# bioinformatics-ua/polus

Measured on AMD Instinct MI355X. Metric: train samples/sec BioBERT-base NER seq256, higher is better.
Workload: dtype bf16; 1 GPU; BERT-base (L=12,H=768,A=12,I=3072,V=28996) token classification C=4, seq_len=256, 64 samples/GPU, AdamW lr 5e-5 wd 0.01 warm-up 10%, dropout 0.1 (hidden + attention) (BASELINE.json configs[2] per-GPU shape), random-init weights; global_batch=64, seq_len=256, parallelism=dp1, grad_allreduce=none

## Files before the change

polus_amd/csrc/common.h:

```cpp
#pragma once
#include <hip/hip_runtime.h>
#include <stdint.h>
#include <stdio.h>
#include <string.h>
#include <math.h>

#include "../../include/polus_hip.h"

typedef __bf16 bf16_t;
typedef __bf16 bf16x8 __attribute__((ext_vector_type(8)));
typedef __bf16 bf16x4 __attribute__((ext_vector_type(4)));
typedef short s16x4 __attribute__((ext_vector_type(4)));
typedef float f32x4 __attribute__((ext_vector_type(4)));

void polus_set_error(const char* fmt, ...);
#define POLUS_FAIL(...) do { polus_set_error(__VA_ARGS__); return POLUS_ERR_INVALID; } while (0)
#define POLUS_REQUIRE(cond, ...) do { if (!(cond)) { polus_set_error(__VA_ARGS__); return POLUS_ERR_INVALID; } } while (0)
#define POLUS_CHECK_LAUNCH(name) do { hipError_t e__ = hipGetLastError(); \
    if (e__ != hipSuccess) { polus_set_error("%s: launch failed: %s", name, hipGetErrorString(e__)); return POLUS_ERR_HIP; } } while (0)
#define POLUS_HIP(call) do { hipError_t e__ = (call); \
    if (e__ != hipSuccess) { polus_set_error("%s failed: %s", #call, hipGetErrorString(e__)); return POLUS_ERR_HIP; } } while (0)

template <auto Kern, typename... A>
int polus_launch_lds(const char* who, dim3 grid, dim3 block, size_t lds_max, size_t lds, hipStream_t st, const A&... args) {
    static bool attr_done = false;
    if (!attr_done) {
        POLUS_HIP(hipFuncSetAttribute(reinterpret_cast<const void*>(Kern), hipFuncAttributeMaxDynamicSharedMemorySize, (int)lds_max));
        attr_done = true;
    }
    hipLaunchKernelGGL(Kern, grid, block, lds, st, args...);
    POLUS_CHECK_LAUNCH(who);
    return POLUS_OK;
}

static inline size_t polus_dtype_size(int dt) { return dt == POLUS_BF16 ? 2 : 4; }
static inline bool polus_aligned16(const void* p) { return (((uintptr_t)p) & 15) == 0; }

struct PolusCfg {
    int gemm_pp;
    int gemm_v1;
    int dw_ungrouped;
    int dw_fused_reduce;
    int ln_bwd_blocks;
    int ln_fin_single;
    int gemm_ring128;
    int gemm_auto_split;
    int ln_halfwave;
    int gemm_order;
    int gemm_persist;
    int reserve_cus;
    int attn_bwd_kres;
    int attn_debug;
    int attn_kskip;
    int dw_streamk;
    int dw_sk_cus;
    int dw_sk_delta;
    int attn_fused;
};
const PolusCfg& polus_cfg();
int polus_num_cus();
int polus_reserved_cus();

struct PolusDyn { uint32_t salt; float lr, lr_t; uint32_t pad; };
const PolusDyn* polus_dyn();
__device__ __forceinline__ uint32_t polus_eff_seed(uint32_t seed, const PolusDyn* dyn) {
    if (!dyn) return seed;
    uint32_t x = seed + dyn->salt;
    x ^= x >> 15;
    return x * 0x2C1B3C6Du;
}

template <typename T> __device__ __forceinline__ float to_f(T x);
template <> __device__ __forceinline__ float to_f<float>(float x) { return x; }
template <> __device__ __forceinline__ float to_f<bf16_t>(bf16_t x) { return (float)x; }
template <typename T> __device__ __forceinline__ T from_f(float x);
template <> __device__ __forceinline__ float from_f<float>(float x) { return x; }
template <> __device__ __forceinline__ bf16_t from_f<bf16_t>(float x) { return (bf16_t)x; }

template <typename T> __device__ __forceinline__ void load4(const T* p, float (&v)[4]);
template <> __device__ __forceinline__ void load4<float>(const float* p, float (&v)[4]) {
    float4 t = *reinterpret_cast<const float4*>(p); v[0] = t.x; v[1] = t.y; v[2] = t.z; v[3] = t.w;
}
template <> __device__ __forceinline__ void load4<bf16_t>(const bf16_t* p, float (&v)[4]) {
    bf16x4 t = *reinterpret_cast<const bf16x4*>(p);
    v[0] = (float)t[0]; v[1] = (float)t[1]; v[2] = (float)t[2]; v[3] = (float)t[3];
}
template <typename T> __device__ __forceinline__ void store4(T* p, const float (&v)[4]);
template <> __device__ __forceinline__ void store4<float>(float* p, const float (&v)[4]) {
    *reinterpret_cast<float4*>(p) = make_float4(v[0], v[1], v[2], v[3]);
}
template <> __device__ __forceinline__ void store4<bf16_t>(bf16_t* p, const float (&v)[4]) {
    bf16x4 t; t[0] = (bf16_t)v[0]; t[1] = (bf16_t)v[1]; t[2] = (bf16_t)v[2]; t[3] = (bf16_t)v[3];
    *reinterpret_cast<bf16x4*>(p) = t;
}

__device__ __forceinline__ float erf_fast(float x) {
    const float ax = fabsf(x);
    const float t = __frcp_rn(1.0f + 0.3275911f * ax);
    float poly = 1.061405429f;
    poly = poly * t - 1.453152027f;
    poly = poly * t + 1.421413741f;
    poly = poly * t - 0.284496736f;
    poly = poly * t + 0.254829592f;
    const float r = 1.0f - poly * t * __expf(-ax * ax);
    return copysignf(r, x);
}
__device__ __forceinline__ float gelu_f(float x) { return 0.5f * x * (1.0f + erf_fast(x * 0.70710678118654752f)); }
__device__ __forceinline__ float gelu_grad_f(float x) {
    float cdf = 0.5f * (1.0f + erf_fast(x * 0.70710678118654752f));
    float pdf = 0.3989422804014327f * __expf(-0.5f * x * x);
    return cdf + x * pdf;
}
__device__ __forceinline__ float swish_f(float x) { return x / (1.0f + __expf(-x)); }
__device__ __forceinline__ float swish_grad_f(float x) {
    float s = 1.0f / (1.0f + __expf(-x));
    return s * (1.0f + x * (1.0f - s));
}
typedef float f32x2_t __attribute__((ext_vector_type(2)));
__device__ __forceinline__ f32x2_t gelu_poly2(f32x2_t x, const float (&c)[11]) {
    f32x2_t xc = {__builtin_amdgcn_fmed3f(x[0], -4.5f, 4.5f), __builtin_amdgcn_fmed3f(x[1], -4.5f, 4.5f)};
    f32x2_t s = xc * xc;
    f32x2_t u = __builtin_elementwise_fma(s, (f32x2_t){2.0f / 20.25f, 2.0f / 20.25f}, (f32x2_t){-1.0f, -1.0f});
    f32x2_t r = {c[10], c[10]};
#pragma unroll
    for (int k = 9; k >= 0; --k) r = __builtin_elementwise_fma(r, u, (f32x2_t){c[k], c[k]});
    return __builtin_elementwise_fma(xc, r, (f32x2_t){0.5f, 0.5f});
}
__device__ __forceinline__ f32x2_t gelu_cdf2(f32x2_t x) {
    const float q[11] = {1.569049305e-01f, -7.719386095e-02f, 5.470119065e-02f, -4.010921159e-02f, 2.828393083e-02f,
                         -1.902094059e-02f, 1.143922652e-02f, -5.251548121e-03f, 2.716277400e-03f, -2.340015935e-03f,
                         9.806926012e-04f};
    return gelu_poly2(x, q);
}
__device__ __forceinline__ f32x2_t gelu_grad2(f32x2_t x) {
    const float w[11] = {1.594289755e-01f, -9.003904569e-02f, 8.714168751e-02f, -9.350841452e-02f, 9.645831298e-02f,
                         -9.557466143e-02f, 7.437658385e-02f, -3.356380937e-02f, 2.252388123e-02f, -3.068672777e-02f,
                         1.457471506e-02f};
    return gelu_poly2(x, w);
}
template <int N, bool FAST = false> __device__ __forceinline__ void apply_act_n(int act, float (&v)[N]) {
    if (act == POLUS_ACT_GELU) {
        if (FAST && (N % 2) == 0) {
#pragma unroll
            for (int r = 0; r < N; r += 2) {
                f32x2_t x = {v[r], v[r + 1]};
                f32x2_t y = x * gelu_cdf2(x);
                v[r] = y[0]; v[r + 1] = y[1];
            }
            return;
        }
#pragma unroll
        for (int r = 0; r < N; ++r) v[r] = gelu_f(v[r]);
    } else if (act == POLUS_ACT_SWISH) {
#pragma unroll
        for (int r = 0; r < N; ++r) v[r] = swish_f(v[r]);
    } else if (act == POLUS_ACT_RELU) {
#pragma unroll
        for (int r = 0; r < N; ++r) v[r] = fmaxf(v[r], 0.0f);
    } else if (act == POLUS_ACT_TANH) {
#pragma unroll
        for (int r = 0; r < N; ++r) v[r] = tanhf(v[r]);
    }
}
template <int N, bool FAST = false> __device__ __forceinline__ void apply_act_grad_n(int act, float (&v)[N], const float (&u)[N]) {
    if (act == POLUS_ACT_GELU) {
        if (FAST && (N % 2) == 0) {
#pragma unroll
            for (int r = 0; r < N; r += 2) {
                f32x2_t d = (f32x2_t){v[r], v[r + 1]} * gelu_grad2((f32x2_t){u[r], u[r + 1]});
                v[r] = d[0]; v[r + 1] = d[1];
            }
            return;
        }
#pragma unroll
        for (int r = 0; r < N; ++r) v[r] *= gelu_grad_f(u[r]);
    } else if (act == POLUS_ACT_SWISH) {
#pragma unroll
        for (int r = 0; r < N; ++r) v[r] *= swish_grad_f(u[r]);
    } else if (act == POLUS_ACT_RELU) {
#pragma unroll
        for (int r = 0; r < N; ++r) v[r] = u[r] > 0.0f ? v[r] : 0.0f;
    } else if (act == POLUS_ACT_TANH) {
#pragma unroll
        for (int r = 0; r < N; ++r) { float t = tanhf(u[r]); v[r] *= 1.0f - t * t; }
    }
}

__device__ __forceinline__ uint32_t polus_hash32(uint32_t seed, uint32_t idx) {
    uint32_t x = idx * 0x9E3779B1u + seed;
    x ^= x >> 16; x *= 0x85EBCA6Bu;
    x ^= x >> 13; x *= 0xC2B2AE35u;
    x ^= x >> 16;
    return x;
}
__device__ __forceinline__ uint32_t polus_hash32_second(uint32_t h1) {
    uint32_t y = h1 * 0x27D4EB2Fu;
    return y ^ (y >> 15);
}
__device__ __forceinline__ bool polus_keep(uint32_t seed, uint32_t idx, uint32_t thresh) {
    const uint32_t h1 = polus_hash32(seed, idx >> 2);
    const uint32_t h = (idx & 2u) ? polus_hash32_second(h1) : h1;
    return ((idx & 1u) ? (h >> 16) : (h & 0xFFFFu)) >= thresh;
}
__device__ __forceinline__ void polus_keep4(uint32_t seed, uint32_t idx4, uint32_t thresh, bool (&k)[4]) {
    const uint32_t h1 = polus_hash32(seed, idx4 >> 2), h2 = polus_hash32_second(h1);
    k[0] = (h1 & 0xFFFFu) >= thresh;
    k[1] = (h1 >> 16) >= thresh;
    k[2] = (h2 & 0xFFFFu) >= thresh;
    k[3] = (h2 >> 16) >= thresh;
}
template <int N>
__device__ __forceinline__ void polus_dropout_run(float (&v)[N], uint32_t seed, uint32_t base, uint32_t thresh, float inv, bool quad) {
    static_assert(N % 4 == 0, "runs of whole quads");
    if (quad) {
#pragma unroll
        for (int r = 0; r < N; r += 4) {
            bool k[4];
            polus_keep4(seed, base + r, thresh, k);
#pragma unroll
            for (int e = 0; e < 4; ++e) v[r + e] = k[e] ? v[r + e] * inv : 0.f;
        }
    } else {
#pragma unroll
        for (int r = 0; r < N; ++r) v[r] = polus_keep(seed, base + r, thresh) ? v[r] * inv : 0.f;
    }
}
static inline uint32_t polus_drop_thresh(float p) {
    double t = (double)p * 65536.0 + 0.5;
    return t <= 0.0 ? 0u : (t >= 65535.0 ? 65535u : (uint32_t)t);
}

__device__ __forceinline__ float wave_sum(float v) {
#pragma unroll
    for (int o = 32; o > 0; o >>= 1) v += __shfl_xor(v, o, 64);
    return v;
}
__device__ __forceinline__ float wave_max(float v) {
#pragma unroll
    for (int o = 32; o > 0; o >>= 1) v = fmaxf(v, __shfl_xor(v, o, 64));
    return v;
}

template <typename T> struct Frag;
template <> struct Frag<bf16_t> { bf16x8 v; };
template <> struct Frag<float> { float v[8]; };

__device__ __forceinline__ void mma16(f32x4& acc, const Frag<bf16_t>& a, const Frag<bf16_t>& b) {
    acc = __builtin_amdgcn_mfma_f32_16x16x32_bf16(a.v, b.v, acc, 0, 0, 0);
}
__device__ __forceinline__ void mma16(f32x4& acc, const Frag<float>& a, const Frag<float>& b) {
#pragma unroll
    for (int j = 0; j < 8; ++j) acc = __builtin_amdgcn_mfma_f32_16x16x4f32(a.v[j], b.v[j], acc, 0, 0, 0);
}

typedef __attribute__((address_space(3))) s16x4 lds_s16x4;

__device__ __forceinline__ void frag_load_row(Frag<bf16_t>& f, const unsigned char* p) {
    f.v = *reinterpret_cast<const bf16x8*>(p);
}
__device__ __forceinline__ void frag_load_row(Frag<float>& f, const unsigned char* p) {
    float4 a = *reinterpret_cast<const float4*>(p);
    float4 b = *reinterpret_cast<const float4*>(p + 16);
    f.v[0] = a.x; f.v[1] = a.y; f.v[2] = a.z; f.v[3] = a.w;
    f.v[4] = b.x; f.v[5] = b.y; f.v[6] = b.z; f.v[7] = b.w;
}

__device__ __forceinline__ s16x4 lds_tr16(const unsigned char* p) {
    return __builtin_amdgcn_ds_read_tr16_b64_v4i16((lds_s16x4*)(p));
}
```

polus_amd/csrc/embed.hip:

```cpp
#include "rowwise.h"

namespace {

template <int NC>
__device__ __forceinline__ void gather_sum(const float* word, const float* pos, const float* type, int id, int s,
                                           int tt, int H, int lane, float (&v)[NC][4]) {
    const float* w = word + (long)id * H;
    const float* p = pos + (long)s * H;
    const float* t = type + (long)tt * H;
#pragma unroll
    for (int c = 0; c < NC; ++c) {
        int col = (lane + 64 * c) * 4;
        if (col < H) {
            float a[4], b[4], d[4];
            load4<float>(w + col, a); load4<float>(p + col, b); load4<float>(t + col, d);
#pragma unroll
            for (int e = 0; e < 4; ++e) v[c][e] = (a[e] + d[e]) + b[e];
        } else { v[c][0] = v[c][1] = v[c][2] = v[c][3] = 0.f; }
    }
}

template <typename T, int NC>
__global__ __launch_bounds__(LN_THREADS) void embed_fwd_kernel(const int32_t* __restrict__ ids, const int32_t* __restrict__ tts,
                                                        const float* __restrict__ word, const float* __restrict__ pos,
                                                        const float* __restrict__ type, const float* __restrict__ gamma,
                                                        const float* __restrict__ beta, T* __restrict__ y,
                                                        float* __restrict__ mean, float* __restrict__ rstd,
                                                        int B, int S, int H, int vocab, int type_vocab, float eps,
                                                        unsigned dthresh, unsigned dseed, float dinv, const PolusDyn* dyn) {
    if (dthresh) dseed = polus_eff_seed(dseed, dyn);
    const int lane = threadIdx.x & 63, wid = threadIdx.x >> 6;
    const int rows = B * S;
    float gv[NC][4], bv[NC][4];
    load_feat<NC>(gamma, H, lane, gv);
    load_feat<NC>(beta, H, lane, bv);
    for (int row = blockIdx.x * WAVES + wid; row < rows; row += gridDim.x * WAVES) {
        const int id = clamp_id(ids[row], vocab);
        const int tt = clamp_id(tts ? tts[row] : 0, type_vocab);
        float v[NC][4];
        gather_sum<NC>(word, pos, type, id, row % S, tt, H, lane, v);
        float mu, rs;
        row_stats<NC>(v, H, lane, eps, mu, rs);
        normalize_store<T, NC>(v, gv, bv, y + (long)row * H, H, lane, mu, rs, dthresh, dseed, dinv, (unsigned)row * (unsigned)H);
        if (lane == 0) { mean[row] = mu; rstd[row] = rs; }
    }
}

template <typename T, int NC>
__global__ __launch_bounds__(LN_THREADS) void embed_bwd_ln_kernel(const T* __restrict__ dy, const int32_t* __restrict__ ids,
                                                           const int32_t* __restrict__ tts, const float* __restrict__ word,
                                                           const float* __restrict__ pos, const float* __restrict__ type,
                                                           const float* __restrict__ gamma, const float* __restrict__ mean,
                                                           const float* __restrict__ rstd, float* __restrict__ de,
                                                           float* __restrict__ partial, int B, int S, int H, int vocab,
                                                           int type_vocab, DropArgs in_drop) {
    if (in_drop.thresh) in_drop.seed = polus_eff_seed(in_drop.seed, in_drop.dyn);
    extern __shared__ __attribute__((aligned(16))) unsigned char smem_raw[];
    float* lds = reinterpret_cast<float*>(smem_raw);
    const int lane = threadIdx.x & 63, wid = threadIdx.x >> 6;
    const int rows = B * S;
    ColAcc<NC> acc;
    colacc_zero(acc);
    float gv[NC][4];
    load_feat<NC>(gamma, H, lane, gv);
    for (int row = blockIdx.x * WAVES + wid; row < rows; row += gridDim.x * WAVES) {
        const int id = clamp_id(ids[row], vocab);
        const int tt = clamp_id(tts ? tts[row] : 0, type_vocab);
        float xv[NC][4];
        gather_sum<NC>(word, pos, type, id, row % S, tt, H, lane, xv);
        ln_bwd_row<T, float, NC>(xv, dy + (long)row * H, gv, de + (long)row * H, H, lane, mean[row], rstd[row], acc, 0,
                                 nullptr, DropArgs{0, 0, 1.f}, in_drop, (unsigned)row * (unsigned)H);
    }
    colacc_flush(acc, lds, partial, H, lane, wid, 0);
}

constexpr int SC_RUN = 8, SC_WAVES = 8;
template <int NC>
__global__ __launch_bounds__(64 * SC_WAVES) void embed_scatter_atomic_kernel(const float* __restrict__ de, const int32_t* __restrict__ ids,
                                                                      float* __restrict__ gword, int rows, int H, int vocab) {
    const int lane = threadIdx.x & 63, wid = threadIdx.x >> 6;
    const long stride = (long)gridDim.x * SC_WAVES * SC_RUN;
    for (long r0 = ((long)blockIdx.x * SC_WAVES + wid) * SC_RUN; r0 < rows; r0 += stride) {
        int mine = -1;
        if (lane < SC_RUN && r0 + lane < rows) mine = clamp_id(ids[r0 + lane], vocab);
        float row[SC_RUN][NC][4];
#pragma unroll
        for (int j = 0; j < SC_RUN; ++j) {
            const bool valid = r0 + j < rows;
            const float* src = de + (r0 + j) * H + lane;
#pragma unroll
            for (int c = 0; c < NC; ++c)
#pragma unroll
                for (int k = 0; k < 4; ++k)
                    row[j][c][k] = (valid && c * 256 + k * 64 + lane < H) ? src[c * 256 + k * 64] : 0.f;
        }
#pragma unroll
        for (int t = 0; t < SC_RUN; ++t) {
            const int id = __shfl(mine, t, 64);
            const unsigned same = (unsigned)__ballot(mine == id);
            if (id < 0 || (same & ((1u << t) - 1u))) continue;
            float* dst = gword + (long)id * H + lane;
#pragma unroll
            for (int c = 0; c < NC; ++c)
#pragma unroll
                for (int k = 0; k < 4; ++k) {
                    float acc = row[t][c][k];
#pragma unroll
                    for (int j = t + 1; j < SC_RUN; ++j)
                        if ((same >> j) & 1u) acc += row[j][c][k];
                    if (c * 256 + k * 64 + lane < H) atomicAdd(dst + c * 256 + k * 64, acc);
                }
        }
    }
}
__global__ __launch_bounds__(LN_THREADS) void embed_scatter_atomic_wide_kernel(const float* __restrict__ de, const int32_t* __restrict__ ids,
                                                                        float* __restrict__ gword, int rows, int H, int vocab) {
    const int lane = threadIdx.x & 63, wid = threadIdx.x >> 6;
    for (int row = blockIdx.x * WAVES + wid; row < rows; row += gridDim.x * WAVES) {
        const int id = clamp_id(ids[row], vocab);
        const float* src = de + (long)row * H;
        float* dst = gword + (long)id * H;
        for (int col = lane; col < H; col += 64) atomicAdd(dst + col, src[col]);
    }
}

__global__ __launch_bounds__(LN_THREADS) void embed_scatter_owner_kernel(const float* __restrict__ de, const int32_t* __restrict__ ids,
                                                                  float* __restrict__ gword, int rows, int H, int vocab) {
    const int lane = threadIdx.x & 63, wid = threadIdx.x >> 6;
    for (int row = blockIdx.x * WAVES + wid; row < rows; row += gridDim.x * WAVES) {
        auto clampid = [vocab](int v) { return clamp_id(v, vocab); };
        const int cid = clampid(ids[row]);
        bool dup = false;
        for (int j0 = 0; j0 < row && !dup; j0 += 64) {
            int j = j0 + lane;
            bool hit = (j < row) && (clampid(ids[j]) == cid);
            dup = __any(hit);
        }
        if (dup) continue;
        float* dst = gword + (long)cid * H;
        for (int c0 = 0; c0 < H; c0 += 64 * 4) {
            int col = c0 + lane * 4;
            float a[4] = {0.f, 0.f, 0.f, 0.f};
            for (int j0 = row; j0 < rows; j0 += 64) {
                int j = j0 + lane;
                unsigned long long m = __ballot((j < rows) && (clampid(ids[j]) == cid));
                while (m) {
                    int b = __ffsll((long long)m) - 1;
                    m &= m - 1;
                    if (col < H) {
                        float v[4];
                        load4<float>(de + (long)(j0 + b) * H + col, v);
#pragma unroll
                        for (int e = 0; e < 4; ++e) a[e] += v[e];
                    }
                }
            }
            if (col < H) {
                float o[4];
                load4<float>(dst + col, o);
#pragma unroll
                for (int e = 0; e < 4; ++e) o[e] += a[e];
                store4<float>(dst + col, o);
            }
        }
    }
}

__global__ __launch_bounds__(256) void embed_pos_grad_kernel(const float* __restrict__ de, float* __restrict__ gpos,
                                                             int B, int S, int H, int accumulate) {
    long idx = (long)blockIdx.x * blockDim.x + threadIdx.x;
    if (idx >= (long)S * H) return;
    float s = 0.f;
    for (int b = 0; b < B; ++b) s += de[(long)b * S * H + idx];
    gpos[idx] = accumulate ? gpos[idx] + s : s;
}

}

extern "C" size_t polus_embed_bwd_workspace_bytes(int B, int S, int H) {
    size_t rows = (size_t)B * S;
    size_t de = rows * H * sizeof(float);
    size_t part = polus_layernorm_bwd_workspace_bytes((int)rows, H);
    size_t cs = polus_colsum_workspace_bytes((int)rows, H);
    return de + (part > cs ? part : cs) + 256;
}

extern "C" int polus_embed_ln_fwd(int dtype, const int32_t* ids, const int32_t* type_ids,
                                  const float* word, const float* pos, const float* type,
                                  const float* gamma, const float* beta, void* y, float* mean, float* rstd,
                                  int B, int S, int H, int vocab, int max_pos, int type_vocab, float eps,
                                  float drop_p, uint32_t seed, void* stream) {
    POLUS_REQUIRE(ids && word && pos && type && gamma && beta && y && mean && rstd, "polus_embed_ln_fwd: null pointer");
    POLUS_REQUIRE(rowwise_drop_ok(drop_p, (long)B * S, H), "polus_embed_ln_fwd: bad drop_p");
    POLUS_REQUIRE(B > 0 && S > 0 && S <= max_pos, "polus_embed_ln_fwd: S=%d exceeds max_position_embeddings=%d", S, max_pos);
    POLUS_REQUIRE(rowwise_shape_ok((long)B * S, H) && vocab > 0 && type_vocab > 0, "polus_embed_ln_fwd: bad H=%d", H);
    POLUS_REQUIRE(polus_aligned16(word) && polus_aligned16(pos) && polus_aligned16(type) && polus_aligned16(y) &&
                  polus_aligned16(gamma) && polus_aligned16(beta), "polus_embed_ln_fwd: pointers must be 16-byte aligned");
    hipStream_t st = static_cast<hipStream_t>(stream);
    const DropArgs d = drop_args(drop_p, seed);
    const dim3 grid(row_blocks(B * S));
    POLUS_REQUIRE(dtype == POLUS_BF16 || dtype == POLUS_F32, "polus_embed_ln_fwd: bad dtype");
    for_dtype_chunks<1, 2, 3, 4, 8>(dtype, chunks256(H), [&](auto t, auto nc) {
        using T = decltype(t);
        hipLaunchKernelGGL((embed_fwd_kernel<T, nc()>), grid, dim3(LN_THREADS), 0, st, ids, type_ids, word, pos, type, gamma, beta, (T*)y, mean, rstd, B, S, H, vocab, type_vocab, eps, d.thresh, d.seed, d.inv, d.dyn);
    });
    POLUS_CHECK_LAUNCH("polus_embed_ln_fwd");
    return POLUS_OK;
}

extern "C" int polus_embed_ln_bwd(int dtype, const void* dy, const int32_t* ids, const int32_t* type_ids,
                                  const float* word, const float* pos, const float* type, const float* gamma,
                                  const float* mean, const float* rstd,
                                  float* gword, float* gpos, float* gtype, float* ggamma, float* gbeta,
                                  int accumulate, int deterministic,
                                  int B, int S, int H, int vocab, int max_pos, int type_vocab,
                                  float drop_p, uint32_t seed,
                                  void* workspace, size_t workspace_bytes, void* stream) {
    POLUS_REQUIRE(dy && ids && word && pos && type && gamma && mean && rstd && gword && gpos && gtype && ggamma && gbeta,
                  "polus_embed_ln_bwd: null pointer");
    POLUS_REQUIRE(rowwise_drop_ok(drop_p, (long)B * S, H), "polus_embed_ln_bwd: bad drop_p");
    POLUS_REQUIRE(B > 0 && S > 0 && S <= max_pos && rowwise_shape_ok((long)B * S, H), "polus_embed_ln_bwd: bad shape");
    POLUS_REQUIRE(polus_aligned16(dy) && polus_aligned16(gword) && polus_aligned16(workspace),
                  "polus_embed_ln_bwd: pointers must be 16-byte aligned");
    size_t need = polus_embed_bwd_workspace_bytes(B, S, H);
    if (!workspace || workspace_bytes < need) { polus_set_error("polus_embed_ln_bwd: workspace %zu < %zu", workspace_bytes, need); return POLUS_ERR_WORKSPACE; }
    hipStream_t st = static_cast<hipStream_t>(stream);
    const DropArgs in_drop = drop_args(drop_p, seed);
    const int rows = B * S;
    float* de = static_cast<float*>(workspace);
    size_t de_bytes = ((size_t)rows * H * sizeof(float) + 255) / 256 * 256;
    float* partial = reinterpret_cast<float*>(static_cast<unsigned char*>(workspace) + de_bytes);
    size_t partial_bytes = workspace_bytes - de_bytes;
    const int blocks = ln_blocks(rows);
    const size_t lds = 3 * (size_t)H * sizeof(float);
    POLUS_REQUIRE(dtype == POLUS_BF16 || dtype == POLUS_F32, "polus_embed_ln_bwd: bad dtype");
    for_dtype_chunks<1, 2, 3, 4, 8>(dtype, chunks256(H), [&](auto t, auto nc) {
        using T = decltype(t);
        hipLaunchKernelGGL((embed_bwd_ln_kernel<T, nc()>), dim3(blocks), dim3(LN_THREADS), lds, st, (const T*)dy, ids, type_ids, word, pos, type, gamma, mean, rstd, de, partial, B, S, H, vocab, type_vocab, in_drop);
    });
    POLUS_CHECK_LAUNCH("polus_embed_ln_bwd(ln)");
    int rc = polus_ln_finalize(partial, blocks, H, 0, ggamma, gbeta, nullptr, accumulate, 1, st, "polus_embed_ln_bwd(finalize)");
    if (rc != POLUS_OK) return rc;

    if (!accumulate) {
        POLUS_HIP(hipMemsetAsync(gword, 0, (size_t)vocab * H * sizeof(float), st));
        POLUS_HIP(hipMemsetAsync(gpos, 0, (size_t)max_pos * H * sizeof(float), st));
    }
    const int route = scatter_route(H, deterministic);
    if (route == SCATTER_OWNER)
        hipLaunchKernelGGL(embed_scatter_owner_kernel, dim3(row_blocks(rows)), dim3(LN_THREADS), 0, st, de, ids, gword, rows, H, vocab);
    else if (route == SCATTER_WIDE)
        hipLaunchKernelGGL(embed_scatter_atomic_wide_kernel, dim3(row_blocks(rows)), dim3(LN_THREADS), 0, st, de, ids, gword, rows, H, vocab);
    else
        for_chunks<1, 2, 3, 4>(route, [&](auto nc) {
            hipLaunchKernelGGL(embed_scatter_atomic_kernel<nc()>, dim3(capped_blocks(rows, SC_RUN * SC_WAVES, ROW_GRID_CAP)), dim3(64 * SC_WAVES), 0, st, de, ids, gword, rows, H, vocab);
        });
    POLUS_CHECK_LAUNCH("polus_embed_ln_bwd(scatter)");
    hipLaunchKernelGGL(embed_pos_grad_kernel, dim3(((long)S * H + 255) / 256), dim3(256), 0, st, de, gpos, B, S, H, accumulate);
    POLUS_CHECK_LAUNCH("polus_embed_ln_bwd(pos)");
    for (int t = 0; t < type_vocab; ++t) {
        if (type_ids || t == 0) {
            rc = polus_colsum_launch(POLUS_F32, de, H, rows, H, gtype + (long)t * H, accumulate, type_ids, t, partial, partial_bytes, st);
            if (rc != POLUS_OK) return rc;
        } else if (!accumulate) {
            POLUS_HIP(hipMemsetAsync(gtype + (long)t * H, 0, (size_t)H * sizeof(float), st));
        }
    }
    return POLUS_OK;
}
```

polus_amd/csrc/runtime.hip:

```cpp
#include "common.h"
#include <stdarg.h>

static thread_local char g_err[512] = "";

void polus_set_error(const char* fmt, ...) {
    va_list ap;
    va_start(ap, fmt);
    vsnprintf(g_err, sizeof(g_err), fmt, ap);
    va_end(ap);
}

extern "C" const char* polus_last_error(void) { return g_err; }

static PolusCfg g_cfg;
static bool g_cfg_ready = false;
static int env_int(const char* name, int dflt) {
    const char* e = getenv(name);
    return (e && *e) ? atoi(e) : dflt;
}
static void read_cfg() {
    g_cfg.gemm_pp = env_int("POLUS_GEMM_PP", 0);
    g_cfg.gemm_v1 = getenv("POLUS_GEMM_V1") != nullptr;
    g_cfg.dw_ungrouped = getenv("POLUS_DW_UNGROUPED") != nullptr;
    g_cfg.gemm_order = env_int("POLUS_GEMM_ORDER", 4);
    g_cfg.reserve_cus = env_int("POLUS_GEMM_RESERVE_CUS", 0);
    g_cfg.gemm_persist = env_int("POLUS_GEMM_PERSIST", 1);
    g_cfg.dw_fused_reduce = env_int("POLUS_DW_FUSED_REDUCE", 1);
    g_cfg.attn_fused = env_int("POLUS_ATTN_FUSED", 1);
    g_cfg.attn_bwd_kres = env_int("POLUS_ATTN_BWD_KRES", 1);
    g_cfg.attn_debug = env_int("POLUS_ATTN_DEBUG", 0);
    g_cfg.attn_kskip = env_int("POLUS_ATTN_KSKIP", 1);
    g_cfg.ln_halfwave = env_int("POLUS_LN_HALFWAVE", 1);
    g_cfg.gemm_auto_split = env_int("POLUS_GEMM_AUTO_SPLIT", 1);
    g_cfg.gemm_ring128 = env_int("POLUS_GEMM_RING128", 0);
    g_cfg.ln_bwd_blocks = env_int("POLUS_LN_BWD_BLOCKS", 512);
    g_cfg.ln_fin_single = env_int("POLUS_LN_FIN_SINGLE", 512);
    g_cfg.dw_streamk = env_int("POLUS_DW_STREAMK", 0);
    g_cfg.dw_sk_delta = env_int("POLUS_DW_SK_DELTA", 2);
    g_cfg.dw_sk_cus = env_int("POLUS_DW_SK_CUS", 0);
    g_cfg_ready = true;
}
const PolusCfg& polus_cfg() {
    if (!g_cfg_ready) read_cfg();
    return g_cfg;
}
extern "C" int polus_reload_env(void) { read_cfg(); return POLUS_OK; }

int polus_num_cus() {
    static int n = 0;
    if (!n) {
        int dev = 0; hipDeviceProp_t prop;
        if (hipGetDevice(&dev) == hipSuccess && hipGetDeviceProperties(&prop, dev) == hipSuccess) n = prop.multiProcessorCount;
        if (n <= 0) n = 256;
    }
    return n;
}
static int g_reserve_on = 1;
extern "C" int polus_set_reserve_active(int on) { g_reserve_on = on != 0; return POLUS_OK; }
int polus_reserved_cus() { return g_reserve_on ? polus_cfg().reserve_cus : 0; }

static const PolusDyn* g_dyn = nullptr;
const PolusDyn* polus_dyn() { return g_dyn; }
extern "C" int polus_set_dynamic_params(const void* dev_block16) {
    POLUS_REQUIRE(dev_block16 == nullptr || polus_aligned16(dev_block16), "polus_set_dynamic_params: the block must be 16-byte aligned");
    g_dyn = static_cast<const PolusDyn*>(dev_block16);
    return POLUS_OK;
}
extern "C" int polus_abi_version(void) { return POLUS_ABI_VERSION; }

extern "C" int polus_device_info(int* n_cu, int* lds_bytes_per_cu, char* arch, int arch_len) {
    int dev = 0;
    POLUS_HIP(hipGetDevice(&dev));
    hipDeviceProp_t prop;
    POLUS_HIP(hipGetDeviceProperties(&prop, dev));
    if (n_cu) *n_cu = prop.multiProcessorCount;
    if (lds_bytes_per_cu) *lds_bytes_per_cu = (int)prop.maxSharedMemoryPerMultiProcessor;
    if (arch && arch_len > 0) {
        strncpy(arch, prop.gcnArchName, arch_len - 1);
        arch[arch_len - 1] = 0;
    }
    return POLUS_OK;
}

namespace {

template <typename S, typename D>
__global__ void cast_kernel(const S* __restrict__ src, D* __restrict__ dst, int64_t n) {
    int64_t i4 = ((int64_t)blockIdx.x * blockDim.x + threadIdx.x) * 4;
    const int64_t stride = (int64_t)gridDim.x * blockDim.x * 4;
    for (; i4 < n; i4 += stride) {
        if (i4 + 4 <= n) {
            float v[4];
            load4<S>(src + i4, v);
            store4<D>(dst + i4, v);
        } else {
            for (int64_t j = i4; j < n; ++j) dst[j] = from_f<D>(to_f<S>(src[j]));
        }
    }
}

__global__ void scale_kernel(float* __restrict__ x, float a, int64_t n) {
    int64_t i4 = ((int64_t)blockIdx.x * blockDim.x + threadIdx.x) * 4;
    const int64_t stride = (int64_t)gridDim.x * blockDim.x * 4;
    for (; i4 < n; i4 += stride) {
        if (i4 + 4 <= n) {
            float4 v = *reinterpret_cast<float4*>(x + i4);
            v.x *= a; v.y *= a; v.z *= a; v.w *= a;
            *reinterpret_cast<float4*>(x + i4) = v;
        } else {
            for (int64_t j = i4; j < n; ++j) x[j] *= a;
        }
    }
}

template <typename T>
__global__ void act_bwd_kernel(const T* __restrict__ dy, const T* __restrict__ u, T* __restrict__ du, int64_t n, int act) {
    int64_t i4 = ((int64_t)blockIdx.x * blockDim.x + threadIdx.x) * 4;
    const int64_t stride = (int64_t)gridDim.x * blockDim.x * 4;
    for (; i4 < n; i4 += stride) {
        if (i4 + 4 <= n) {
            float a[4], b[4];
            load4<T>(dy + i4, a);
            load4<T>(u + i4, b);
            apply_act_grad_n<4>(act, a, b);
            store4<T>(du + i4, a);
        } else {
            for (int64_t j = i4; j < n; ++j) { float a1[1] = {to_f<T>(dy[j])}, b1[1] = {to_f<T>(u[j])}; apply_act_grad_n<1>(act, a1, b1); du[j] = from_f<T>(a1[0]); }
        }
    }
}

__global__ __launch_bounds__(256) void transpose16_kernel(const unsigned short* __restrict__ src,
                                                         unsigned short* __restrict__ dst, int R, int C) {
    __shared__ unsigned short tile[64][66];
    const int r0 = blockIdx.y * 64, c0 = blockIdx.x * 64;
    const int tx = threadIdx.x & 63, ty = threadIdx.x >> 6;
    for (int k = ty; k < 64; k += 4) {
        int r = r0 + k, c = c0 + tx;
        tile[k][tx] = (r < R && c < C) ? src[(long)r * C + c] : (unsigned short)0;
    }
    __syncthreads();
    for (int k = ty; k < 64; k += 4) {
        int c = c0 + k, r = r0 + tx;
        if (c < C && r < R) dst[(long)c * R + r] = tile[tx][k];
    }
}

__global__ __launch_bounds__(256) void transpose16_batched_kernel(const unsigned short* __restrict__ src,
                                                                 unsigned short* __restrict__ dst,
                                                                 const long* __restrict__ segs, int nseg) {
    __shared__ unsigned short tile[64][66];
    const int b = blockIdx.x;
    int s = 0;
    while (s + 1 < nseg && segs[4 * (s + 1) + 3] <= b) ++s;
    const long off = segs[4 * s];
    const int R = (int)segs[4 * s + 1], C = (int)segs[4 * s + 2];
    const int t = b - (int)segs[4 * s + 3], tc = (C + 63) / 64;
    const int r0 = (t / tc) * 64, c0 = (t % tc) * 64;
    const unsigned short* sp = src + off;
    unsigned short* dp = dst + off;
    if (((R | C) & 3) == 0) {
        const int q = threadIdx.x & 15, rr = threadIdx.x >> 4;
#pragma unroll
        for (int k = 0; k < 4; ++k) {
            const int r = r0 + rr + 16 * k, c = c0 + 4 * q;
            ushort4 v = make_ushort4(0, 0, 0, 0);
            if (r < R && c < C) v = *reinterpret_cast<const ushort4*>(sp + (long)r * C + c);
            tile[rr + 16 * k][4 * q] = v.x; tile[rr + 16 * k][4 * q + 1] = v.y;
            tile[rr + 16 * k][4 * q + 2] = v.z; tile[rr + 16 * k][4 * q + 3] = v.w;
        }
        __syncthreads();
#pragma unroll
        for (int k = 0; k < 4; ++k) {
            const int c = c0 + rr + 16 * k, r = r0 + 4 * q;
            if (c < C && r < R) {
                ushort4 v = make_ushort4(tile[4 * q][rr + 16 * k], tile[4 * q + 1][rr + 16 * k],
                                         tile[4 * q + 2][rr + 16 * k], tile[4 * q + 3][rr + 16 * k]);
                *reinterpret_cast<ushort4*>(dp + (long)c * R + r) = v;
            }
        }
        return;
    }
    const int tx = threadIdx.x & 63, ty = threadIdx.x >> 6;
    for (int k = ty; k < 64; k += 4) {
        int r = r0 + k, c = c0 + tx;
        tile[k][tx] = (r < R && c < C) ? sp[(long)r * C + c] : (unsigned short)0;
    }
    __syncthreads();
    for (int k = ty; k < 64; k += 4) {
        int c = c0 + k, r = r0 + tx;
        if (c < C && r < R) dp[(long)c * R + r] = tile[tx][k];
    }
}

template <typename T>
__global__ void dropout_kernel(const T* __restrict__ x, T* __restrict__ y, int64_t n, unsigned seed, unsigned thresh, float inv,
                               const PolusDyn* dyn) {
    seed = polus_eff_seed(seed, dyn);
    int64_t i = (int64_t)blockIdx.x * blockDim.x + threadIdx.x;
    const int64_t stride = (int64_t)gridDim.x * blockDim.x;
    for (; i < n; i += stride) y[i] = polus_keep(seed, (unsigned)i, thresh) ? from_f<T>(to_f<T>(x[i]) * inv) : from_f<T>(0.f);
}

__global__ void dropout_mask_kernel(unsigned seed, unsigned thresh, unsigned idx0, int64_t n, uint8_t* __restrict__ mask,
                                    const PolusDyn* dyn) {
    seed = polus_eff_seed(seed, dyn);
    int64_t i = (int64_t)blockIdx.x * blockDim.x + threadIdx.x;
    const int64_t stride = (int64_t)gridDim.x * blockDim.x;
    for (; i < n; i += stride) mask[i] = polus_keep(seed, idx0 + (unsigned)i, thresh) ? 1 : 0;
}

inline int stream_grid(int64_t n) {
    int64_t b = (n / 4 + 255) / 256;
    if (b < 1) b = 1;
    if (b > 2048) b = 2048;
    return (int)b;
}

}

extern "C" int polus_cast(int src_dtype, const void* src, int dst_dtype, void* dst, int64_t n, void* stream) {
    POLUS_REQUIRE(src && dst && n >= 0, "polus_cast: bad arguments");
    if (n == 0) return POLUS_OK;
    POLUS_REQUIRE(((uintptr_t)src % (4 * polus_dtype_size(src_dtype))) == 0 &&
                  ((uintptr_t)dst % (4 * polus_dtype_size(dst_dtype))) == 0,
                  "polus_cast: pointers must be 4-element aligned");
    hipStream_t st = static_cast<hipStream_t>(stream);
    dim3 grid(stream_grid(n)), block(256);
    if (src_dtype == POLUS_F32 && dst_dtype == POLUS_BF16)
        hipLaunchKernelGGL((cast_kernel<float, bf16_t>), grid, block, 0, st, (const float*)src, (bf16_t*)dst, n);
    else if (src_dtype == POLUS_BF16 && dst_dtype == POLUS_F32)
        hipLaunchKernelGGL((cast_kernel<bf16_t, float>), grid, block, 0, st, (const bf16_t*)src, (float*)dst, n);
    else if (src_dtype == POLUS_F32 && dst_dtype == POLUS_F32)
        hipLaunchKernelGGL((cast_kernel<float, float>), grid, block, 0, st, (const float*)src, (float*)dst, n);
    else if (src_dtype == POLUS_BF16 && dst_dtype == POLUS_BF16)
        hipLaunchKernelGGL((cast_kernel<bf16_t, bf16_t>), grid, block, 0, st, (const bf16_t*)src, (bf16_t*)dst, n);
    else POLUS_FAIL("polus_cast: bad dtypes %d -> %d", src_dtype, dst_dtype);
    POLUS_CHECK_LAUNCH("polus_cast");
    return POLUS_OK;
}

extern "C" int polus_scale(float* x, float a, int64_t n, void* stream) {
    POLUS_REQUIRE(x && n >= 0, "polus_scale: bad arguments");
    if (n == 0) return POLUS_OK;
    POLUS_REQUIRE(((uintptr_t)x % 16) == 0, "polus_scale: pointer must be 16-byte aligned");
    hipLaunchKernelGGL(scale_kernel, dim3(stream_grid(n)), dim3(256), 0, static_cast<hipStream_t>(stream), x, a, n);
    POLUS_CHECK_LAUNCH("polus_scale");
    return POLUS_OK;
}

extern "C" int polus_act_bwd(int dtype, const void* dy, const void* u, void* du, int64_t n, int act, void* stream) {
    POLUS_REQUIRE(dy && u && du && n >= 0, "polus_act_bwd: bad arguments");
    if (n == 0) return POLUS_OK;
    size_t es = polus_dtype_size(dtype);
    POLUS_REQUIRE(((uintptr_t)dy % (4 * es)) == 0 && ((uintptr_t)u % (4 * es)) == 0 && ((uintptr_t)du % (4 * es)) == 0,
                  "polus_act_bwd: pointers must be 4-element aligned");
    hipStream_t st = static_cast<hipStream_t>(stream);
    if (dtype == POLUS_BF16)
        hipLaunchKernelGGL(act_bwd_kernel<bf16_t>, dim3(stream_grid(n)), dim3(256), 0, st, (const bf16_t*)dy, (const bf16_t*)u, (bf16_t*)du, n, act);
    else if (dtype == POLUS_F32)
        hipLaunchKernelGGL(act_bwd_kernel<float>, dim3(stream_grid(n)), dim3(256), 0, st, (const float*)dy, (const float*)u, (float*)du, n, act);
    else POLUS_FAIL("polus_act_bwd: bad dtype");
    POLUS_CHECK_LAUNCH("polus_act_bwd");
    return POLUS_OK;
}

extern "C" int polus_transpose_bf16_batched(const void* src_base, void* dst_base, const void* segs_dev, int nseg,
                                            int total_tiles, void* stream) {
    POLUS_REQUIRE(src_base && dst_base && segs_dev && nseg > 0 && total_tiles > 0, "polus_transpose_bf16_batched: bad arguments");
    POLUS_REQUIRE(((uintptr_t)src_base % 8) == 0 && ((uintptr_t)dst_base % 8) == 0,
                  "polus_transpose_bf16_batched: the arenas must be 8-byte aligned");
    hipLaunchKernelGGL(transpose16_batched_kernel, dim3(total_tiles), dim3(256), 0, static_cast<hipStream_t>(stream),
                       (const unsigned short*)src_base, (unsigned short*)dst_base, (const long*)segs_dev, nseg);
    POLUS_CHECK_LAUNCH("polus_transpose_bf16_batched");
    return POLUS_OK;
}

extern "C" int polus_transpose_bf16(const void* src, void* dst, int rows, int cols, void* stream) {
    POLUS_REQUIRE(src && dst && rows > 0 && cols > 0, "polus_transpose_bf16: bad arguments");
    dim3 grid((cols + 63) / 64, (rows + 63) / 64);
    hipLaunchKernelGGL(transpose16_kernel, grid, dim3(256), 0, static_cast<hipStream_t>(stream),
                       (const unsigned short*)src, (unsigned short*)dst, rows, cols);
    POLUS_CHECK_LAUNCH("polus_transpose_bf16");
    return POLUS_OK;
}

extern "C" int polus_dropout_mask(uint32_t seed, float drop_p, uint32_t idx0, int64_t n, uint8_t* mask, void* stream) {
    POLUS_REQUIRE(mask && n >= 0 && drop_p >= 0.0f && drop_p < 1.0f, "polus_dropout_mask: bad arguments");
    if (n == 0) return POLUS_OK;
    int64_t b = (n + 255) / 256;
    if (b > 4096) b = 4096;
    hipLaunchKernelGGL(dropout_mask_kernel, dim3((int)b), dim3(256), 0, static_cast<hipStream_t>(stream),
                       seed, polus_drop_thresh(drop_p), idx0, n, mask, polus_dyn());
    POLUS_CHECK_LAUNCH("polus_dropout_mask");
    return POLUS_OK;
}

extern "C" int polus_dropout(int dtype, const void* x, void* y, int64_t n, float drop_p, uint32_t seed, void* stream) {
    POLUS_REQUIRE(x && y && n >= 0 && n < (1LL << 32) && drop_p >= 0.0f && drop_p < 1.0f, "polus_dropout: bad arguments");
    if (n == 0) return POLUS_OK;
    int64_t b = (n + 255) / 256;
    if (b > 4096) b = 4096;
    hipStream_t st = static_cast<hipStream_t>(stream);
    const unsigned th = drop_p > 0.f ? polus_drop_thresh(drop_p) : 0u;
    const float inv = 1.0f / (1.0f - drop_p);
    if (dtype == POLUS_BF16) hipLaunchKernelGGL(dropout_kernel<bf16_t>, dim3((int)b), dim3(256), 0, st, (const bf16_t*)x, (bf16_t*)y, n, seed, th, inv, polus_dyn());
    else if (dtype == POLUS_F32) hipLaunchKernelGGL(dropout_kernel<float>, dim3((int)b), dim3(256), 0, st, (const float*)x, (float*)y, n, seed, th, inv, polus_dyn());
    else POLUS_FAIL("polus_dropout: bad dtype");
    POLUS_CHECK_LAUNCH("polus_dropout");
    return POLUS_OK;
}
```

Measured before the change: 5360 samples/s.

## Fuse embedding LayerNorm backward with word, position and type gradient scatter

Adds a single fused kernel that recomputes the embedding sum, runs the LayerNorm backward in registers, and scatters word gradients with atomics. The same kernel also accumulates position gradients with a per-position running sum across the batch and keeps type-gradient partials in LDS. This removes the fp32 de workspace round trip, the separate scatter, position-grad and colsum kernels, and the gpos memset. The cost is a more complex kernel with per-wave serialized __syncthreads loops, a different atomic summation order, and a dependence on rows being assigned to blocks by position. It is enabled by default through an env flag.

```diff
diff --git a/polus_amd/csrc/common.h b/polus_amd/csrc/common.h
--- a/polus_amd/csrc/common.h
+++ b/polus_amd/csrc/common.h
@@ -46,6 +46,7 @@
     int gemm_ring128;
     int gemm_auto_split;
     int ln_halfwave;
+    int embed_bwd_fused;
     int gemm_order;
     int gemm_persist;
     int reserve_cus;
diff --git a/polus_amd/csrc/embed.hip b/polus_amd/csrc/embed.hip
--- a/polus_amd/csrc/embed.hip
+++ b/polus_amd/csrc/embed.hip
@@ -163,6 +163,197 @@
                 store4<float>(dst + col, o);
             }
         }
+    }
+}
+
+template <int NC>
+__device__ __forceinline__ void ln_bwd_row_regs(const float (&xv)[NC][4], float (&dy)[NC][4], const float (&gv)[NC][4],
+                                                int H, int lane, float mu, float rs, ColAcc<NC>& acc,
+                                                DropArgs in_drop, unsigned rowbase, float (&o)[NC][4]) {
+    if (in_drop.thresh) {
+#pragma unroll
+        for (int c = 0; c < NC; ++c) {
+            int col = (lane + 64 * c) * 4;
+            polus_dropout_run<4>(dy[c], in_drop.seed, rowbase + col, in_drop.thresh, in_drop.inv, true);
+        }
+    }
+    float s1 = 0.f, s2 = 0.f;
+    float xh[NC][4], dxh[NC][4];
+#pragma unroll
+    for (int c = 0; c < NC; ++c) {
+        int col = (lane + 64 * c) * 4;
+        if (col < H) {
+#pragma unroll
+            for (int e = 0; e < 4; ++e) {
+                xh[c][e] = (xv[c][e] - mu) * rs;
+                dxh[c][e] = dy[c][e] * gv[c][e];
+                s1 += dxh[c][e];
+                s2 += dxh[c][e] * xh[c][e];
+                acc.dg[c][e] += dy[c][e] * xh[c][e];
+                acc.db[c][e] += dy[c][e];
+            }
+        } else {
+#pragma unroll
+            for (int e = 0; e < 4; ++e) xh[c][e] = dxh[c][e] = 0.f;
+        }
+    }
+    s1 = wave_sum(s1) / (float)H;
+    s2 = wave_sum(s2) / (float)H;
+#pragma unroll
+    for (int c = 0; c < NC; ++c) {
+        int col = (lane + 64 * c) * 4;
+#pragma unroll
+        for (int e = 0; e < 4; ++e) o[c][e] = col < H ? (dxh[c][e] - s1 - xh[c][e] * s2) * rs : 0.f;
+    }
+}
+
+constexpr int FB_WAVES = 8, FB_TYPES = 4;
+constexpr int fb_run(int nc, int raw) { return nc * (4 + raw) <= 18 ? 8 : (nc * (4 + raw) <= 24 ? 4 : 2); }
+inline size_t fb_lds_bytes(int H, int type_vocab) { return ((size_t)(4 + type_vocab) * H + FB_WAVES * 256) * sizeof(float); }
+template <typename T, int NC>
+__global__ __launch_bounds__(64 * FB_WAVES) void embed_bwd_fused_kernel(const T* __restrict__ dy, const int32_t* __restrict__ ids,
+                                                                 const int32_t* __restrict__ tts, const float* __restrict__ word,
+                                                                 const float* __restrict__ pos, const float* __restrict__ type,
+                                                                 const float* __restrict__ gamma, const float* __restrict__ mean,
+                                                                 const float* __restrict__ rstd, float* __restrict__ gword,
+                                                                 float* __restrict__ gpos, float* __restrict__ partial,
+                                                                 float* __restrict__ tpartial, int B, int S, int H, int vocab,
+                                                                 int max_pos, int type_vocab, int accumulate, DropArgs in_drop) {
+    using Raw = std::conditional_t<std::is_same_v<T, float>, f32x4, bf16x4>;
+    constexpr int R = fb_run(NC, sizeof(Raw) / 4);
+    if (in_drop.thresh) in_drop.seed = polus_eff_seed(in_drop.seed, in_drop.dyn);
+    extern __shared__ __attribute__((aligned(16))) unsigned char smem_raw[];
+    float* lds = reinterpret_cast<float*>(smem_raw);
+    const int lane = threadIdx.x & 63, wid = threadIdx.x >> 6;
+    float* posacc = lds + 3 * H;
+    float* typeacc = posacc + H;
+    float* stage = typeacc + (long)type_vocab * H + wid * 256;
+    for (int idx = threadIdx.x; idx < type_vocab * H; idx += blockDim.x) typeacc[idx] = 0.f;
+    if (!accumulate)
+        for (long idx = (long)S * H + (long)blockIdx.x * blockDim.x + threadIdx.x; idx < (long)max_pos * H; idx += (long)gridDim.x * blockDim.x)
+            gpos[idx] = 0.f;
+    __syncthreads();
+    ColAcc<NC> acc;
+    colacc_zero(acc);
+    float gv[NC][4];
+    load_feat<NC>(gamma, H, lane, gv);
+    const int npos = (int)blockIdx.x < S ? (S - 1 - (int)blockIdx.x) / (int)gridDim.x + 1 : 0;
+    const int n = npos * B;
+    for (int c0 = 0; c0 < n; c0 += FB_WAVES * R) {
+        int row_l = -1, id_l = -1, tt_l = 0, b_l = 0, s_l = 0;
+        float mu_l = 0.f, rs_l = 0.f;
+        if (lane < R && c0 + wid * R + lane < n) {
+            const int i = c0 + wid * R + lane;
+            b_l = i % B; s_l = blockIdx.x + (i / B) * gridDim.x; row_l = b_l * S + s_l;
+            id_l = clamp_id(ids[row_l], vocab); tt_l = clamp_id(tts ? tts[row_l] : 0, type_vocab);
+            mu_l = mean[row_l]; rs_l = rstd[row_l];
+        }
+        float de[R][NC][4];
+        Raw dyr[R][NC];
+#pragma unroll
+        for (int j = 0; j < R; ++j) {
+            const int row = __builtin_amdgcn_readlane(row_l, j);
+            const float* w = word + (long)__builtin_amdgcn_readlane(id_l, j) * H;
+            const T* d = dy + (long)row * H;
+#pragma unroll
+            for (int c = 0; c < NC; ++c) {
+                const int col = (lane + 64 * c) * 4;
+                if (row >= 0 && col < H) {
+                    load4<float>(w + col, de[j][c]);
+                    dyr[j][c] = *reinterpret_cast<const Raw*>(d + col);
+                } else {
+                    de[j][c][0] = de[j][c][1] = de[j][c][2] = de[j][c][3] = 0.f;
+                    dyr[j][c] = Raw{};
+                }
+            }
+        }
+#pragma unroll
+        for (int j = 0; j < R; ++j) {
+            const int row = __builtin_amdgcn_readlane(row_l, j);
+            if (row < 0) continue;
+            const float* p = pos + (long)__builtin_amdgcn_readlane(s_l, j) * H;
+            const float* t = type + (long)__builtin_amdgcn_readlane(tt_l, j) * H;
+            float xv[NC][4], dyv[NC][4];
+#pragma unroll
+            for (int c = 0; c < NC; ++c) {
+                const int col = (lane + 64 * c) * 4;
+                if (col < H) {
+                    float b[4], d[4];
+                    load4<float>(p + col, b); load4<float>(t + col, d);
+#pragma unroll
+                    for (int e = 0; e < 4; ++e) xv[c][e] = (de[j][c][e] + d[e]) + b[e];
+                } else { xv[c][0] = xv[c][1] = xv[c][2] = xv[c][3] = 0.f; }
+#pragma unroll
+                for (int e = 0; e < 4; ++e) dyv[c][e] = (float)dyr[j][c][e];
+            }
+            ln_bwd_row_regs<NC>(xv, dyv, gv, H, lane, __int_as_float(__builtin_amdgcn_readlane(__float_as_int(mu_l), j)),
+                                __int_as_float(__builtin_amdgcn_readlane(__float_as_int(rs_l), j)), acc, in_drop,
+                                (unsigned)row * (unsigned)H, de[j]);
+        }
+#pragma unroll
+        for (int t = 0; t < R; ++t) {
+            const int id = __builtin_amdgcn_readlane(id_l, t);
+            const unsigned same = (unsigned)__ballot(id_l == id);
+            if (id < 0 || (same & ((1u << t) - 1u))) continue;
+            float* dst = gword + (long)id * H + lane;
+#pragma unroll
+            for (int c = 0; c < NC; ++c) {
+                float a[4] = {de[t][c][0], de[t][c][1], de[t][c][2], de[t][c][3]};
+#pragma unroll
+                for (int j = t + 1; j < R; ++j)
+                    if ((same >> j) & 1u) {
+#pragma unroll
+                        for (int e = 0; e < 4; ++e) a[e] += de[j][c][e];
+                    }
+                __builtin_amdgcn_fence(__ATOMIC_ACQ_REL, "wavefront");
+                *reinterpret_cast<float4*>(stage + lane * 4) = make_float4(a[0], a[1], a[2], a[3]);
+                __builtin_amdgcn_fence(__ATOMIC_ACQ_REL, "wavefront");
+#pragma unroll
+                for (int k = 0; k < 4; ++k) {
+                    const float v = stage[k * 64 + lane];
+                    if (c * 256 + k * 64 + lane < H) atomicAdd(dst + c * 256 + k * 64, v);
+                }
+            }
+        }
+        for (int w = 0; w < FB_WAVES; ++w) {
+            if (wid == w) {
+                float run[NC][4];
+#pragma unroll
+                for (int j = 0; j < R; ++j) {
+                    const int row = __builtin_amdgcn_readlane(row_l, j);
+                    if (row < 0) continue;
+                    const int b = __builtin_amdgcn_readlane(b_l, j), s = __builtin_amdgcn_readlane(s_l, j);
+                    float* ta = typeacc + (long)__builtin_amdgcn_readlane(tt_l, j) * H;
+#pragma unroll
+                    for (int c = 0; c < NC; ++c) {
+                        const int col = (lane + 64 * c) * 4;
+                        if (col >= H) continue;
+                        float4 tv = *reinterpret_cast<float4*>(ta + col);
+                        tv.x += de[j][c][0]; tv.y += de[j][c][1]; tv.z += de[j][c][2]; tv.w += de[j][c][3];
+                        *reinterpret_cast<float4*>(ta + col) = tv;
+                        if (b == 0) { run[c][0] = run[c][1] = run[c][2] = run[c][3] = 0.f; }
+                        else if (j == 0) { const float4 pv = *reinterpret_cast<float4*>(posacc + col); run[c][0] = pv.x; run[c][1] = pv.y; run[c][2] = pv.z; run[c][3] = pv.w; }
+#pragma unroll
+                        for (int e = 0; e < 4; ++e) run[c][e] += de[j][c][e];
+                        if (b == B - 1) {
+                            float* g = gpos + (long)s * H + col;
+#pragma unroll
+                            for (int e = 0; e < 4; ++e) g[e] = accumulate ? g[e] + run[c][e] : run[c][e];
+                        } else if (j == R - 1) {
+                            *reinterpret_cast<float4*>(posacc + col) = make_float4(run[c][0], run[c][1], run[c][2], run[c][3]);
+                        }
+                    }
+                }
+            }
+            __syncthreads();
+        }
+    }
+    colacc_flush(acc, lds, partial, H, lane, wid, 0);
+    float* p0 = partial + (long)blockIdx.x * 3 * H + 2 * H;
+    float* p1 = tpartial + (long)blockIdx.x * 3 * H;
+    for (int idx = threadIdx.x; idx < type_vocab * H; idx += blockDim.x) {
+        if (idx < H) p0[idx] = typeacc[idx];
+        else p1[idx - H] = typeacc[idx];
     }
 }
 
@@ -234,6 +425,22 @@
     const int blocks = ln_blocks(rows);
     const size_t lds = 3 * (size_t)H * sizeof(float);
     POLUS_REQUIRE(dtype == POLUS_BF16 || dtype == POLUS_F32, "polus_embed_ln_bwd: bad dtype");
+    const int route = scatter_route(H, deterministic);
+    if (polus_cfg().embed_bwd_fused && route <= 4 && type_vocab <= FB_TYPES) {
+        float* fpartial = static_cast<float*>(workspace);
+        float* tpartial = fpartial + (size_t)blocks * 3 * H;
+        POLUS_REQUIRE((size_t)blocks * 6 * H * sizeof(float) <= workspace_bytes, "polus_embed_ln_bwd: workspace too small for the partial sums");
+        if (!accumulate) POLUS_HIP(hipMemsetAsync(gword, 0, (size_t)vocab * H * sizeof(float), st));
+        for_dtype_chunks<1, 2, 3, 4>(dtype, route, [&](auto t, auto nc) {
+            using T = decltype(t);
+            hipLaunchKernelGGL((embed_bwd_fused_kernel<T, nc()>), dim3(blocks), dim3(64 * FB_WAVES), fb_lds_bytes(H, type_vocab), st, (const T*)dy, ids, type_ids, word, pos, type, gamma, mean, rstd, gword, gpos, fpartial, tpartial, B, S, H, vocab, max_pos, type_vocab, accumulate, in_drop);
+        });
+        POLUS_CHECK_LAUNCH("polus_embed_ln_bwd(fused)");
+        int rc = polus_ln_finalize(fpartial, blocks, H, 1, ggamma, gbeta, gtype, accumulate, 1, st, "polus_embed_ln_bwd(finalize)");
+        if (rc != POLUS_OK || type_vocab == 1) return rc;
+        return polus_ln_finalize(tpartial, blocks, H, type_vocab > 3, gtype + H, type_vocab > 2 ? gtype + 2 * (long)H : nullptr,
+                                 type_vocab > 3 ? gtype + 3 * (long)H : nullptr, accumulate, 1, st, "polus_embed_ln_bwd(finalize types)");
+    }
     for_dtype_chunks<1, 2, 3, 4, 8>(dtype, chunks256(H), [&](auto t, auto nc) {
         using T = decltype(t);
         hipLaunchKernelGGL((embed_bwd_ln_kernel<T, nc()>), dim3(blocks), dim3(LN_THREADS), lds, st, (const T*)dy, ids, type_ids, word, pos, type, gamma, mean, rstd, de, partial, B, S, H, vocab, type_vocab, in_drop);
@@ -246,7 +453,6 @@
         POLUS_HIP(hipMemsetAsync(gword, 0, (size_t)vocab * H * sizeof(float), st));
         POLUS_HIP(hipMemsetAsync(gpos, 0, (size_t)max_pos * H * sizeof(float), st));
     }
-    const int route = scatter_route(H, deterministic);
     if (route == SCATTER_OWNER)
         hipLaunchKernelGGL(embed_scatter_owner_kernel, dim3(row_blocks(rows)), dim3(LN_THREADS), 0, st, de, ids, gword, rows, H, vocab);
     else if (route == SCATTER_WIDE)
diff --git a/polus_amd/csrc/runtime.hip b/polus_amd/csrc/runtime.hip
--- a/polus_amd/csrc/runtime.hip
+++ b/polus_amd/csrc/runtime.hip
@@ -31,7 +31,8 @@
     g_cfg.attn_debug = env_int("POLUS_ATTN_DEBUG", 0);
     g_cfg.attn_kskip = env_int("POLUS_ATTN_KSKIP", 1);
     g_cfg.ln_halfwave = env_int("POLUS_LN_HALFWAVE", 1);
-    g_cfg.gemm_auto_split = env_int("POLUS_GEMM_AUTO_SPLIT", 1);
+    g_cfg.embed_bwd_fused = env_int("POLUS_EMBED_BWD_FUSED", 1);
+    g_cfg.gemm_auto_split =env_int("POLUS_GEMM_AUTO_SPLIT", 1);
     g_cfg.gemm_ring128 = env_int("POLUS_GEMM_RING128", 0);
     g_cfg.ln_bwd_blocks = env_int("POLUS_LN_BWD_BLOCKS", 512);
     g_cfg.ln_fin_single = env_int("POLUS_LN_FIN_SINGLE", 512);
```

Result: no change. 5387 samples/s, median of 6 (+0.5%).
